# leaxer-ai/leaxer-qwen3-tts

Measured on AMD Instinct MI355X. Metric: real-time factor (24 kHz audio sec / wall sec), Qwen3-TTS-0.6B, higher is better.
Workload: dtype bf16 weights, fp32 activations/accumulate (codec decoder: fp16 hi/lo split operands, fp32 accumulate)

## Files before the change

### leaxer-qwen3-tts_amd/csrc/q3_common.h

```cpp
#pragma once
#include <hip/hip_runtime.h>
#include <stdint.h>
#include <string>

#include "../../include/q3tts.h"

typedef uint16_t bf16_t;

#define Q3_HIP_CHECK(expr)                                                                         \
    do {                                                                                           \
        hipError_t _e = (expr);                                                                    \
        if (_e != hipSuccess) throw q3::Error(std::string(#expr) + ": " + hipGetErrorString(_e));  \
    } while (0)

namespace q3 {

struct Error {
    std::string msg;
    explicit Error(std::string m) : msg(std::move(m)) {}
};

const char* knob(const char* name);
struct KnobScope {
    bool on = false;
// ... 28 lines not shown
    int ld_xn = 0;
    const float* bias = nullptr;
    const float* res = nullptr;
    int ldres = 0;
    float* out = nullptr;
    int ldo = 0;
    int M = 0, N = 0, K = 0;
    int epi = EPI_STORE;
    bool nt = false;
    const float* po = nullptr;
    const float* pm = nullptr;
    const float* pl = nullptr;
    int pS = 0, pchunk = 0, pn_new = 1, pslot_offset = 0, pheads = 0, pd = 0;
    const int* ppos_dev = nullptr;
    int ppos_scalar = 0;
};
void launch_gemv(const GemvArgs& a, hipStream_t s);
bool gemv_fast_path(const GemvArgs& a);
bool gemv16_ok(const GemvArgs& a);
void launch_gemv16(const GemvArgs& a, hipStream_t s);
void launch_pack_mfma_b(const bf16_t* W, bf16_t* P, int N, int K, hipStream_t s);
size_t packed_mfma_b_elems(int N, int K);
void register_packed_weight(const bf16_t* W, const bf16_t* P);
void unregister_packed_weight(const bf16_t* W);
const bf16_t* find_packed_weight(const bf16_t* W);

struct AttnArgs {
    const float* qkv = nullptr;
    int ld_qkv = 0;
    const float* ssq_in = nullptr; int ssq_nt = 0, ssq_K = 0; float ssq_eps = 0.f;
// ... 29 lines not shown
void launch_attn(const AttnArgs& a, hipStream_t s);
struct CpAttnOprojArgs {
    const float* qkv = nullptr; int ld_qkv = 0;
    float* kc = nullptr; float* vc = nullptr;
    int page_tokens = 0;
    int base = 0;
    const float* q_norm = nullptr; const float* k_norm = nullptr; float eps = 0.f;
    const float* rope_cos = nullptr; const float* rope_sin = nullptr;
    float scale = 0.f;
    int nq = 0, nkv = 0, d = 0;
    const bf16_t* W = nullptr; int K = 0, N = 0;
    float* x = nullptr; int ldx = 0;
};
bool cp_attn_oproj_ok(const CpAttnOprojArgs& a, int n_new);
void launch_cp_attn_oproj(const CpAttnOprojArgs& a, int n_new, hipStream_t s);
void launch_attn_combine(const AttnArgs& a, hipStream_t s);

struct GemmArgs {
    const bf16_t* W = nullptr;
    const bf16_t* W2 = nullptr;
    const bf16_t* xh = nullptr;
    const bf16_t* xl = nullptr;
    int ldx = 0;
    const float* res = nullptr; int ldres = 0;
    const float* bias = nullptr;
    float* out = nullptr; int ldo = 0;
    float* out2 = nullptr;
    bf16_t* oh = nullptr; bf16_t* ol = nullptr; int ldp = 0;
    int M = 0, N = 0, K = 0, epi = EPI_STORE;
    int slab_rows = 0;
// ... 141 lines not shown
```

### leaxer-qwen3-tts_amd/csrc/q3_decode_kernels.hip

```cpp
#include "q3_common.h"
#include "q3_wave_sort.h"
#include <algorithm>

namespace q3 {

#ifdef Q3_SAMPLE_PROF
__device__ long long g_kernel_prof[32];
void sample_prof_read(long long* out) { (void)hipMemcpyFromSymbol(out, HIP_SYMBOL(g_kernel_prof), sizeof(long long) * 32); }
#define KP_MARK(k) do { if (blockIdx.x == 0 && blockIdx.y == 0 && blockIdx.z == 0 && threadIdx.x == 0) g_kernel_prof[k] = wall_clock64(); } while (0)
#else
#define KP_MARK(k) do { } while (0)
#endif

#define Q3_DPP_XOR1 0xB1
#define Q3_DPP_XOR2 0x4E
#define Q3_DPP_ROR4 0x124
#define Q3_DPP_ROR8 0x128
#define Q3_DPP_BCAST15 0x142
#define Q3_DPP_BCAST31 0x143
template <int CTRL, int ROW_MASK>
static __device__ __forceinline__ float dpp_f(float oldv, float v) {
    return __builtin_bit_cast(float, __builtin_amdgcn_update_dpp(__builtin_bit_cast(int, oldv), __builtin_bit_cast(int, v), CTRL, ROW_MASK, 0xF, false));
}
template <int CTRL, int ROW_MASK>
// ... 183 lines not shown
    const int R = (a.N >= 4096 && a.epi != EPI_SWIGLU) ? 2 : 1;
    int grid = (a.N + 4 * R - 1) / (4 * R);
    if (grid > 2048) grid = 2048;
    if (grid < 1) grid = 1;
    if (R == 2) gemv_epi<MT, 2>(a, grid, s); else gemv_epi<MT, 1>(a, grid, s);
}


static __device__ __forceinline__ uint4 ldw_rt(const bf16_t* p, bool nt) {
    u32x4 v;
    if (nt) v = __builtin_nontemporal_load(reinterpret_cast<const u32x4*>(p));
    else v = *reinterpret_cast<const u32x4*>(p);
    return make_uint4(v.x, v.y, v.z, v.w);
}

template <int MT, int NCH, int RW, int EPI, bool NORM, bool COMB>
__global__ __launch_bounds__(256) void k_gemv1(const bf16_t* pW, const bf16_t* pW2, const float* px, const float* pgamma, const float* pepi,
                                                int pN, int pM, int pldx, int pldepi, int pnt, GemvArgs a) {
    constexpr int K = NCH * 512;
    const int lane = threadIdx.x & 63;
    const int wave = __builtin_amdgcn_readfirstlane(threadIdx.x >> 6);
    const int n0 = (blockIdx.x * 4 + wave) * RW;
    const int N = pN, M = pM;
    __shared__ float xs[COMB ? MT * K : 1];

    KP_MARK(30); KP_MARK(31);
    KP_MARK(8);
    uint4 w[RW][NCH], w2[RW][NCH];
#pragma unroll
    for (int r = 0; r < RW; ++r) {
        const int n = n0 + r < N ? n0 + r : N - 1;
#pragma unroll
        for (int c = 0; c < NCH; ++c) {
            w[r][c] = ldw_rt(pW + (size_t)n * K + c * 512 + lane * 8, pnt != 0);
            if (EPI == EPI_SWIGLU) w2[r][c] = ldw_rt(pW2 + (size_t)n * K + c * 512 + lane * 8, pnt != 0);
        }
    }
    __builtin_amdgcn_sched_barrier(0);
    float epi_in = 0.f;
    if (EPI == EPI_RESIDUAL || EPI == EPI_BIAS || EPI == EPI_BIAS_SILU) {
        if (lane < MT * RW) {
            const int m = lane / RW, n = n0 + lane % RW;
            if (m < M && n < N) epi_in = EPI == EPI_RESIDUAL ? pepi[(size_t)m * pldepi + n] : pepi[n];
        }
    }
    float xv[MT][NCH][8];
    if (COMB) {
        for (int k8 = threadIdx.x * 8; k8 < K; k8 += 2048) {
            const int head = k8 / a.pd, e0 = k8 % a.pd;
#pragma unroll
            for (int m = 0; m < MT; ++m) {
                if (m < M) {
                    const int bi = m / a.pn_new, inew = m % a.pn_new;
                    const int pos = (a.ppos_dev ? a.ppos_dev[a.pslot_offset + bi] : a.ppos_scalar) + inew;
                    int nact = pos / a.pchunk + 1;
                    if (nact > a.pS) nact = a.pS;
                    const size_t idx = ((size_t)m * a.pheads + head) * a.pS;
                    constexpr int CQ = 12;
                    float mx = -INFINITY, L = 0.f, O[8] = {0.f, 0.f, 0.f, 0.f, 0.f, 0.f, 0.f, 0.f};
                    for (int sp0 = 0; sp0 < nact; sp0 += CQ) {
                        float pmv[CQ], plv[CQ];
                        float4 o0[CQ], o1[CQ];
// ... 36 lines not shown
                xv[m][c][0] = x0.x; xv[m][c][1] = x0.y; xv[m][c][2] = x0.z; xv[m][c][3] = x0.w;
                xv[m][c][4] = x1.x; xv[m][c][5] = x1.y; xv[m][c][6] = x1.z; xv[m][c][7] = x1.w;
            }
    } else {
#pragma unroll
        for (int m = 0; m < MT; ++m)
#pragma unroll
            for (int c = 0; c < NCH; ++c) {
                const float* xr = px + (size_t)(m < M ? m : 0) * pldx + c * 512 + lane * 8;
                const float4 x0 = *reinterpret_cast<const float4*>(xr);
                const float4 x1 = *reinterpret_cast<const float4*>(xr + 4);
                xv[m][c][0] = x0.x; xv[m][c][1] = x0.y; xv[m][c][2] = x0.z; xv[m][c][3] = x0.w;
                xv[m][c][4] = x1.x; xv[m][c][5] = x1.y; xv[m][c][6] = x1.z; xv[m][c][7] = x1.w;
            }
    }
    float g[NORM ? NCH : 1][8];
    if (NORM) {
#pragma unroll
        for (int c = 0; c < NCH; ++c) {
            const float4 g0 = *reinterpret_cast<const float4*>(pgamma + c * 512 + lane * 8);
            const float4 g1 = *reinterpret_cast<const float4*>(pgamma + c * 512 + lane * 8 + 4);
            g[c][0] = g0.x; g[c][1] = g0.y; g[c][2] = g0.z; g[c][3] = g0.w; g[c][4] = g1.x; g[c][5] = g1.y; g[c][6] = g1.z; g[c][7] = g1.w;
        }
    }
    KP_MARK(9);
    __builtin_amdgcn_sched_barrier(0);
    if (NORM) {
#pragma unroll
        for (int m = 0; m < MT; ++m) {
            float ss = 0.f;
#pragma unroll
            for (int c = 0; c < NCH; ++c)
#pragma unroll
                for (int j = 0; j < 8; ++j) ss = fmaf(xv[m][c][j], xv[m][c][j], ss);
            ss = wave_sum(ss);
            const float inv = 1.0f / sqrtf(ss / (float)K + a.eps);
#pragma unroll
            for (int c = 0; c < NCH; ++c)
#pragma unroll
// ... 48 lines not shown
static int gemv1_rw(const GemvArgs& a) {
    int rw = a.N / 1024;
    if (rw < 1) rw = 1;
    if (rw > 4) rw = 4;
    if (a.epi == EPI_SWIGLU && rw > 3) rw = 3;
    if (a.K > 3072 && rw > 2) rw = 2;
    return rw;
}
bool gemv_fast_path(const GemvArgs& a) {
    if (a.M < 1 || a.M > 2) return false;
    if (a.K != 1024 && a.K != 2048 && a.K != 3072 && !(a.K == 6144 && a.M == 1)) return false;
    if (a.ldx % 4 != 0 && !a.po) return false;
    const bool norm = a.gamma != nullptr, comb = a.po != nullptr;
    if (comb && (norm || a.epi != EPI_RESIDUAL || a.pd % 8 != 0 || a.pheads * a.pd != a.K)) return false;
    if (norm && a.epi != EPI_STORE && a.epi != EPI_SWIGLU) return false;
    return true;
}

template <int MT, int NCH, int RW>
static void gemv1_launch(const GemvArgs& a, int grid, hipStream_t s) {
    const bool norm = a.gamma != nullptr, comb = a.po != nullptr;
#define Q3_G1(EPI, NORM, COMB) hipLaunchKernelGGL((k_gemv1<MT, NCH, RW, EPI, NORM, COMB>), dim3(grid), dim3(256), 0, s, a.W, a.W2, a.x, a.gamma, \
        (a.epi == EPI_RESIDUAL ? a.res : a.bias), a.N, a.M, a.ldx, a.ldres, (int)a.nt, a)
    if (comb) { Q3_G1(EPI_RESIDUAL, false, true); return; }
    switch (a.epi) {
    case EPI_STORE: if (norm) Q3_G1(EPI_STORE, true, false); else Q3_G1(EPI_STORE, false, false); break;
    case EPI_SWIGLU:
        if constexpr (RW <= 3) { if (norm) Q3_G1(EPI_SWIGLU, true, false); else Q3_G1(EPI_SWIGLU, false, false); }
        else throw Error("gemv: SwiGLU fast path takes at most 3 rows per wave");
        break;
    case EPI_RESIDUAL: Q3_G1(EPI_RESIDUAL, false, false); break;
    case EPI_BIAS: Q3_G1(EPI_BIAS, false, false); break;
    default: Q3_G1(EPI_BIAS_SILU, false, false); break;
    }
#undef Q3_G1
}
template <int MT, int NCH>
static void gemv1_rwsel(const GemvArgs& a, hipStream_t s) {
    const int rw = gemv1_rw(a);
    const int grid = (a.N + 4 * rw - 1) / (4 * rw);
    if (rw == 1) gemv1_launch<MT, NCH, 1>(a, grid, s);
    else if (rw == 2) gemv1_launch<MT, NCH, 2>(a, grid, s);
    else if constexpr (NCH <= 6) {
        if (rw == 3) gemv1_launch<MT, NCH, 3>(a, grid, s);
        else gemv1_launch<MT, NCH, 4>(a, grid, s);
    } else throw Error("gemv: K = 6144 fast path takes at most 2 rows per wave");
}
template <int MT>
static void gemv1_nch(const GemvArgs& a, hipStream_t s) {
    if (a.K == 1024) gemv1_rwsel<MT, 2>(a, s);
// ... 1366 lines not shown

void launch_cp_attn_oproj(const CpAttnOprojArgs& a, int n_new, hipStream_t s) {
    if (!cp_attn_oproj_ok(a, n_new)) throw Error("cp_attn_oproj: unsupported shape");
    const int U = a.base <= 4 ? 1 : (a.base <= 8 ? 2 : (a.base <= 12 ? 3 : 4));
    const dim3 grid((a.N + 3) / 4), block(1024);
#define Q3_CAO(NEW, UU) hipLaunchKernelGGL((k_cp_attn_oproj<NEW, UU>), grid, block, 0, s, a.W, a.qkv, (const float*)a.kc, (const float*)a.vc, (const float*)a.x, \
        a.rope_cos, a.rope_sin, (uint32_t)a.base | (uint32_t)a.page_tokens << 16, (uint32_t)a.N | (uint32_t)a.ldx << 16, a)
    if (n_new == 1) { if (U == 1) Q3_CAO(1, 1); else if (U == 2) Q3_CAO(1, 2); else if (U == 3) Q3_CAO(1, 3); else Q3_CAO(1, 4); }
    else { if (U == 1) Q3_CAO(2, 1); else if (U == 2) Q3_CAO(2, 2); else Q3_CAO(2, 3); }
#undef Q3_CAO
    Q3_HIP_CHECK(hipGetLastError());
}
bool cp_attn_oproj_ok(const CpAttnOprojArgs& a, int n_new) {
    return (n_new == 1 || (n_new == 2 && a.base <= 12)) && a.nq == 16 && a.nkv == 8 && a.d == 128 && a.K == 2048 && a.base >= 0 && a.base <= 16 &&
           a.base + n_new <= a.page_tokens && a.q_norm && a.k_norm && a.ld_qkv == 4096 && a.N >= 1 && a.N < 65536 && a.ldx < 65536 && a.page_tokens < 65536;
}

#define SAMP_MAXV 4096

static __device__ __forceinline__ uint64_t mix64(uint64_t z) {
    z += 0x9E3779B97F4A7C15ull;
    z = (z ^ (z >> 30)) * 0xBF58476D1CE4E5B9ull;
    z = (z ^ (z >> 27)) * 0x94D049BB133111EBull;
    return z ^ (z >> 31);
}
static __device__ __forceinline__ float rng_uniform_dev(uint64_t seed, uint32_t stream, uint32_t frame, uint32_t group) {
    uint64_t k = mix64(seed ^ mix64(((uint64_t)stream << 32) | frame));
    k = mix64(k + group);
    return (float)(k >> 40) * (1.0f / 16777216.0f);
}
// ... 635 lines not shown
```

### leaxer-qwen3-tts_amd/csrc/q3_engine.cpp

```cpp
#include "q3_engine.h"

#include <algorithm>
#include <atomic>
#include <cmath>
#include <cstdio>
#include <cstdlib>
#include <cstring>

namespace q3 {

static const int64_t TTS_BOS = 151672, TTS_EOS = 151673, TTS_PAD = 151671;
static const int64_t CODEC_BOS = 2149, CODEC_PAD = 2148, CODEC_THINK = 2154, CODEC_NOTHINK = 2155;
static const int64_t CODEC_THINK_BOS = 2156, CODEC_THINK_EOS = 2157, LANG_ENGLISH = 2050;

static uint64_t mix64(uint64_t z) {
    z += 0x9E3779B97F4A7C15ull;
    z = (z ^ (z >> 30)) * 0xBF58476D1CE4E5B9ull;
    z = (z ^ (z >> 27)) * 0x94D049BB133111EBull;
    return z ^ (z >> 31);
}
static uint64_t fnv1a(const std::string& s) {
    uint64_t h = 1469598103934665603ull;
    for (unsigned char ch : s) { h ^= ch; h *= 1099511628211ull; }
    return h;
// ... 136 lines not shown
    if (flags & Q3TTS_FLAG_TEST_HOOKS) knob_scope.enable();
    if (B < 1 || B > 1024) throw Error("max_batch out of range");
    if (kv_pool_tokens < 0) throw Error("kv_pool_tokens must be >= 0");
    if (c.cp_hidden < 0) throw Error("cp_hidden must be >= 0");
    if (c.cp_hidden == c.hidden) c.cp_hidden = 0;
    if (c.hidden % 8 || c.ffn % 8 || c.text_hidden % 8 || c.cp_ffn % 8 || cp_width() % 8) throw Error("hidden/ffn sizes must be multiples of 8");
    if (c.vocab > 4096 || c.sub_vocab > 4096) throw Error("codec vocabularies larger than 4096 are not supported");
    if (c.n_groups < 2 || c.n_groups > 32) throw Error("n_groups out of range");
    Q3_HIP_CHECK(hipSetDevice(device));
    if (const char* mr = knob("Q3TTS_MFMA_MIN_ROWS")) mfma_min_rows = std::max(3, atoi(mr));
    if (const char* sv = knob("Q3TTS_SEAM")) seam_on = atoi(sv) != 0;
    if (const char* sv = knob("Q3TTS_SEAM_SPIN")) seam_spin = std::max(1, atoi(sv));
    attn_keep_splits = knob("Q3TTS_ATTN_KEEP_SPLITS") != nullptr;
    if (const char* sv = knob("Q3TTS_ATTN_STREAM")) attn_stream = atoi(sv) != 0;
    if (const char* sv = knob("Q3TTS_ATTN_STREAM_ONE")) attn_stream_one = atoi(sv) != 0;
    null_stream = getenv("Q3TTS_NULL_STREAM") && getenv("Q3TTS_NULL_STREAM")[0] == '1';
    if (null_stream) { stream = nullptr; flags |= Q3TTS_FLAG_NO_GRAPH; }
    else if (const char* cm = knob("Q3TTS_STREAM_CU_MASK")) {
        const uint32_t pat = (uint32_t)strtoul(cm, nullptr, 16);
        if (pat == 0) throw Error("Q3TTS_STREAM_CU_MASK must be a non-zero hexadecimal CU pattern (a stream with no CU never runs)");
        uint32_t mask[8];
        for (int i = 0; i < 8; ++i) mask[i] = pat;
        Q3_HIP_CHECK(hipExtStreamCreateWithCUMask(&stream, 8, mask));
    }
    else {
        int lo = 0, hi = 0;
        Q3_HIP_CHECK(hipDeviceGetStreamPriorityRange(&lo, &hi));
        Q3_HIP_CHECK(hipStreamCreateWithPriority(&stream, hipStreamNonBlocking, hi));
    }
    Q3_HIP_CHECK(hipEventCreate(&ev0));
// ... 46 lines not shown
    x_cp1 = fm((size_t)B * H);
    if (cp_projected()) x_cpp = fm((size_t)std::max(rows_max, 16) * Hc);
    sum = fm((size_t)B * H);
    xp = fm((size_t)std::max(16, rows_max) * H);
    hn = fm((size_t)std::max(16, rows_max) * H);
    logits_p = fm((size_t)16 * std::max(c.vocab, c.sub_vocab));
    trailing_d = fm((size_t)B * max_trailing * H);
    tts_pad_d = fm(H);
    text_tmp = fm((size_t)16 * c.text_hidden);
    text_tmp2 = fm((size_t)16 * c.text_hidden);
    ldp = (std::max(std::max(H, AO), std::max(c.ffn, c.cp_ffn)) + 7) / 8 * 8;
    pl0h = (bf16_t*)dmalloc((size_t)rows_max * ldp * 2); pl0l = (bf16_t*)dmalloc((size_t)rows_max * ldp * 2);
    pl1h = (bf16_t*)dmalloc((size_t)rows_max * ldp * 2); pl1l = (bf16_t*)dmalloc((size_t)rows_max * ldp * 2);
    slab_d = fm((size_t)16 * rows_max * H);
    qkv_slab_d = fm((size_t)4 * rows_max * std::max(QKV, QKVp));
    {
        const size_t per_launch = (size_t)(std::max(std::max(c.ffn, c.cp_ffn), H) / 64 + 1) * 2 * 16;
        const size_t launches = (size_t)3 * ((size_t)c.n_layers + (size_t)(c.n_groups - 1) * c.cp_layers) + 8;
        seam_cnt_words = per_launch * launches;
        seam_cnt_d = (unsigned*)dmalloc(seam_cnt_words * sizeof(unsigned));
        Q3_HIP_CHECK(hipMemsetAsync(seam_cnt_d, 0, seam_cnt_words * sizeof(unsigned), stream));
        seam_gen_d = (unsigned*)dmalloc(64);
        Q3_HIP_CHECK(hipMemsetAsync(seam_gen_d, 0, 64, stream));
        ssq_a_d = fm((size_t)rows_max * 64);
        ssq_b_d = fm((size_t)rows_max * 64);
    }
    gu_slab_d = fm((size_t)2 * 8 * rows_max * std::max(c.ffn, c.cp_ffn));
    ids_d = (int64_t*)dmalloc(64 * sizeof(int64_t));
    tok_d = (int64_t*)dmalloc(sizeof(int64_t));
    codes_d = (int32_t*)dmalloc((size_t)B * max_frames_cap * c.n_groups * sizeof(int32_t));
// ... 249 lines not shown
        } else {
            GemvArgs g;
            g.W = w.qkv; g.x = x; g.ldx = ldx; g.gamma = w.in_norm; g.eps = W.eps; g.out = qkv; g.ldo = QKV;
            g.M = M; g.N = QKV; g.K = W.H; g.epi = EPI_STORE; g.nt = W.nt;
            launch_gemv(g, stream);
        }
        if (!mfma && nb == 1 && pos_dev == nullptr && slot_map == nullptr && W.n_splits == 1 && W.pages_per_slot == 1 && !W.kv_bf16 && !W.kv_round &&
            !(flags & Q3TTS_FLAG_NO_FUSED_CP)) {
            CpAttnOprojArgs f;
            const int ptok = 1 << W.page_shift;
            const size_t coff = (((size_t)slot_offset * W.L + l) * W.nkv) * ptok * W.d;
            f.qkv = qkv; f.ld_qkv = QKV; f.kc = W.kc + coff; f.vc = W.vc + coff; f.page_tokens = ptok; f.base = pos_scalar;
            f.q_norm = w.q_norm; f.k_norm = w.k_norm; f.eps = W.eps; f.rope_cos = W.rope_cos; f.rope_sin = W.rope_sin;
            f.scale = 1.0f / sqrtf((float)W.d); f.nq = W.nq; f.nkv = W.nkv; f.d = W.d; f.W = w.o; f.K = AO; f.N = W.H; f.x = x; f.ldx = ldx;
            if (cp_attn_oproj_ok(f, n_new)) {
                launch_cp_attn_oproj(f, n_new, stream);
                GemvArgs fg;
                fg.W = w.gate; fg.W2 = w.up; fg.x = x; fg.ldx = ldx; fg.gamma = w.post_norm; fg.eps = W.eps; fg.out = act; fg.ldo = W.ffn;
                fg.M = M; fg.N = W.ffn; fg.K = W.H; fg.epi = EPI_SWIGLU; fg.nt = W.nt;
                launch_gemv(fg, stream);
                GemvArgs dg;
                dg.W = w.down; dg.x = act; dg.ldx = W.ffn; dg.res = x; dg.ldres = ldx; dg.out = x; dg.ldo = ldx;
                dg.M = M; dg.N = W.H; dg.K = W.ffn; dg.epi = EPI_RESIDUAL; dg.nt = W.nt;
                launch_gemv(dg, stream);
                continue;
            }
        }
        AttnArgs a;
        a.qkv = qkv; a.ld_qkv = QKV; a.out = attn; a.ld_out = AO; a.kcache = W.kc; a.vcache = W.vc; a.kv_bf16 = W.kv_bf16; a.kv_round = W.kv_round;
        if (mfma) { a.qkv = qkv_slab_d; a.qkv_nslab = ks_q; a.qkv_slab_stride = (size_t)M * QKV; }
        if (seam && (l > 0 || planes_in)) { a.ssq_in = ssq_b_d; a.ssq_nt = NTH; a.ssq_K = W.H; a.ssq_eps = W.eps; }
        a.page_table = W.page_table; a.pages_per_slot = W.pages_per_slot; a.page_shift = W.page_shift; a.identity_pages = W.identity_pages;
        a.layer = l; a.n_layers = W.L; a.q_norm = w.q_norm; a.k_norm = w.k_norm; a.eps = W.eps;
        a.rope_cos = W.rope_cos; a.rope_sin = W.rope_sin; a.pos_dev = pos_dev; a.pos_scalar = pos_scalar;
        a.slot_offset = slot_offset; a.slot_map = slot_map; a.nb = nb; a.n_new = n_new; a.nq = W.nq; a.nkv = W.nkv; a.d = W.d;
        a.scale = 1.0f / sqrtf((float)W.d); a.window = 0; a.new_from_raw = 1;
        a.n_splits = W.n_splits; a.chunk = W.chunk; a.po = W.po; a.pm = W.pm; a.pl = W.pl;
        if (mfma && W.n_splits > 1 && W.identity_pages && !attn_keep_splits && (size_t)nb * W.nkv >= 256 && (W.pages_per_slot << W.page_shift) <= 512) {
// ... 42 lines not shown
                launch_gemm2(d, ks_d, 4, stream);
                continue;
            }
            launch_gemm2(d, ks_d, 4, stream);
            const bool last = l + 1 == W.L;
            const float* ng = last ? final_gamma : W.layers[l + 1].in_norm;
            launch_finish(x, ldx, slab_d, ks_d, (size_t)M * W.H, W.H, ng, last ? final_eps : W.eps, M, W.H, pl0h, pl0l, ldp,
                          last ? final_xn : nullptr, last ? final_ld_xn : 0, stream);
            continue;
        }
        GemvArgs o;
        o.W = w.o; o.x = attn; o.ldx = AO; o.res = x; o.ldres = ldx; o.out = x; o.ldo = ldx;
        o.M = M; o.N = W.H; o.K = AO; o.epi = EPI_RESIDUAL; o.nt = W.nt;
        o.po = W.po; o.pm = W.pm; o.pl = W.pl; o.pS = W.n_splits; o.pchunk = W.chunk; o.pn_new = n_new; o.pslot_offset = slot_offset;
        o.pheads = W.nq; o.pd = W.d; o.ppos_dev = pos_dev; o.ppos_scalar = pos_scalar;
        if (direct_rows) { o.po = nullptr; o.pm = nullptr; o.pl = nullptr; }
        else if (!gemv_fast_path(o)) {
            launch_attn_combine(a, stream);
            o.po = nullptr; o.pm = nullptr; o.pl = nullptr;
        }
        launch_gemv(o, stream);
        GemvArgs f;
        f.W = w.gate; f.W2 = w.up; f.x = x; f.ldx = ldx; f.gamma = w.post_norm; f.eps = W.eps; f.out = act; f.ldo = W.ffn;
        f.M = M; f.N = W.ffn; f.K = W.H; f.epi = EPI_SWIGLU; f.nt = W.nt;
        launch_gemv(f, stream);
        GemvArgs d;
        d.W = w.down; d.x = act; d.ldx = W.ffn; d.res = x; d.ldres = ldx; d.out = x; d.ldo = ldx;
        d.M = M; d.N = W.H; d.K = W.ffn; d.epi = EPI_RESIDUAL; d.nt = W.nt;
        launch_gemv(d, stream);
    }
    return mfma && final_gamma != nullptr;
}

int Engine::head_proj(const bf16_t* Wm, const float* x, int ldx, const float* gamma, float eps, float* xn_out, int ld_xn,
                      float* out, int ldo, int M, int N, int K, bool nt, bool planes_ready, int plane_row0, int plane_row_stride, float* slab_out) {
    if (planes_ready || (M >= mfma_min_rows && K % 128 == 0 && K <= 4096)) {
        if (!planes_ready) {
            launch_finish(const_cast<float*>(x), ldx, nullptr, 0, 0, 0, gamma, eps, M, K, pl0h, pl0l, ldp, xn_out, ld_xn, stream);
            plane_row0 = 0; plane_row_stride = 1;
        }
        GemmArgs g;
        g.W = Wm; g.xh = pl0h + (size_t)plane_row0 * ldp; g.xl = pl0l + (size_t)plane_row0 * ldp; g.ldx = ldp * plane_row_stride;
        g.out = out; g.ldo = ldo; g.M = M; g.N = N; g.K = K; g.epi = EPI_STORE; g.nt = nt;
// ... 824 lines not shown
```

### leaxer-qwen3-tts_amd/csrc/q3_engine.h

```cpp
#pragma once
#include <functional>
#include <memory>
#include <string>
#include <unordered_map>
#include <vector>

#include "q3_common.h"
#include "q3_kvpool.h"

namespace q3 {

enum TensorKind { TK_W = 0, TK_NORM = 1, TK_BIAS = 2, TK_SCALE = 3, TK_SNAKE = 4 };

struct Tensor {
    std::string name;
    int64_t shape[4] = {0, 0, 0, 0};
    int ndim = 0;
    int kind = TK_W;
    bool bf16 = false;
    void* dev = nullptr;
    int64_t numel = 0;
    float synth_std = 0.02f;
};

// ... 174 lines not shown
    float* cp_project(float* rows, int ld, int M);
    std::vector<const bf16_t*> cp_head, cp_embed_w;

    int rows_max = 0, max_trailing = 0, max_frames_cap = 0;
    int mfma_min_rows = 12;
    float *x_talk = nullptr, *qkv = nullptr, *attn = nullptr, *act = nullptr, *logits_t = nullptr, *logits_cp = nullptr;
    float *x_cp = nullptr, *x_cp1 = nullptr, *sum = nullptr, *xp = nullptr, *hn = nullptr, *logits_p = nullptr;
    float *trailing_d = nullptr, *tts_pad_d = nullptr, *text_tmp = nullptr, *text_tmp2 = nullptr;
    int64_t* ids_d = nullptr;
    bf16_t *pl0h = nullptr, *pl0l = nullptr, *pl1h = nullptr, *pl1l = nullptr;
    int ldp = 0;
    float* slab_d = nullptr;
    float* gu_slab_d = nullptr;
    float* cp_logit_slab_d = nullptr;
    float* qkv_slab_d = nullptr;
    unsigned* seam_cnt_d = nullptr; size_t seam_cnt_words = 0, seam_cnt_used = 0;
    unsigned* seam_gen_d = nullptr;
    float *ssq_a_d = nullptr, *ssq_b_d = nullptr;
    bool seam_step = false;
    bool seam_on = true;
    bool attn_stream = true;
    bool attn_stream_one = true;
    bool attn_keep_splits = false;
    int seam_spin = 512;
    int32_t* codes_d = nullptr;
    int32_t* codes_scratch_d = nullptr;
    int32_t* talker_pos_d = nullptr;
    int* slot_map_d = nullptr;
    float* logits_g = nullptr;
    SlotState* st_d = nullptr;
// ... 23 lines not shown
```

Before: 35.90.

## Split o-proj by KV head into partial sums folded into gate/up GEMV prologue

Attention plus o-projection (both the code-predictor fused path and the talker split-combine path) now run with one block per KV-head slice of K and a column chunk. Each writes a per-head partial output vector instead of doing the full K reduction per column inside one block. The following SwiGLU gate/up GEMV gains a prologue that sums the 8 partials with the residual, writes the mid residual for the down projection, and applies RMSNorm. This aims to raise parallelism in the M=1 decode o-proj and remove its serial full-K reduction. The cost is extra partial-buffer traffic and every gate/up block redundantly re-reading the partials.

```diff
diff --git a/leaxer-qwen3-tts_amd/csrc/q3_common.h b/leaxer-qwen3-tts_amd/csrc/q3_common.h
--- a/leaxer-qwen3-tts_amd/csrc/q3_common.h
+++ b/leaxer-qwen3-tts_amd/csrc/q3_common.h
@@ -66,6 +66,8 @@
     int pS = 0, pchunk = 0, pn_new = 1, pslot_offset = 0, pheads = 0, pd = 0;
     const int* ppos_dev = nullptr;
     int ppos_scalar = 0;
+    const float* psum = nullptr;
+    float* xmid = nullptr;
 };
 void launch_gemv(const GemvArgs& a, hipStream_t s);
 bool gemv_fast_path(const GemvArgs& a);
@@ -125,6 +127,9 @@
 };
 bool cp_attn_oproj_ok(const CpAttnOprojArgs& a, int n_new);
 void launch_cp_attn_oproj(const CpAttnOprojArgs& a, int n_new, hipStream_t s);
+void launch_cp_attn_kvh(const CpAttnOprojArgs& a, int n_new, float* part, hipStream_t s);
+bool oproj_kvh_ok(const GemvArgs& a);
+void launch_oproj_kvh(const GemvArgs& a, float* part, hipStream_t s);
 void launch_attn_combine(const AttnArgs& a, hipStream_t s);
 
 struct GemmArgs {
diff --git a/leaxer-qwen3-tts_amd/csrc/q3_decode_kernels.hip b/leaxer-qwen3-tts_amd/csrc/q3_decode_kernels.hip
--- a/leaxer-qwen3-tts_amd/csrc/q3_decode_kernels.hip
+++ b/leaxer-qwen3-tts_amd/csrc/q3_decode_kernels.hip
@@ -221,7 +221,7 @@
     return make_uint4(v.x, v.y, v.z, v.w);
 }
 
-template <int MT, int NCH, int RW, int EPI, bool NORM, bool COMB>
+template <int MT, int NCH, int RW, int EPI, bool NORM, bool COMB, bool PSUM = false>
 __global__ __launch_bounds__(256) void k_gemv1(const bf16_t* pW, const bf16_t* pW2, const float* px, const float* pgamma, const float* pepi,
                                                 int pN, int pM, int pldx, int pldepi, int pnt, GemvArgs a) {
     constexpr int K = NCH * 512;
@@ -229,7 +229,7 @@
     const int wave = __builtin_amdgcn_readfirstlane(threadIdx.x >> 6);
     const int n0 = (blockIdx.x * 4 + wave) * RW;
     const int N = pN, M = pM;
-    __shared__ float xs[COMB ? MT * K : 1];
+    __shared__ float xs[(COMB || PSUM) ? MT * K : 1];
 
     KP_MARK(30); KP_MARK(31);
     KP_MARK(8);
@@ -251,8 +251,56 @@
             if (m < M && n < N) epi_in = EPI == EPI_RESIDUAL ? pepi[(size_t)m * pldepi + n] : pepi[n];
         }
     }
+    float g[NORM ? NCH : 1][8];
+    auto load_gamma = [&]() {
+#pragma unroll
+        for (int c = 0; c < NCH; ++c) {
+            const float4 g0 = *reinterpret_cast<const float4*>(pgamma + c * 512 + lane * 8);
+            const float4 g1 = *reinterpret_cast<const float4*>(pgamma + c * 512 + lane * 8 + 4);
+            g[c][0] = g0.x; g[c][1] = g0.y; g[c][2] = g0.z; g[c][3] = g0.w; g[c][4] = g1.x; g[c][5] = g1.y; g[c][6] = g1.z; g[c][7] = g1.w;
+        }
+    };
     float xv[MT][NCH][8];
-    if (COMB) {
+    if (PSUM) {
+        constexpr int NI = K / 1024, NP = 8;
+        static_assert(K % 1024 == 0, "PSUM: K must be a multiple of 1024");
+        float4 xin[MT][NI], pin[MT][NI][NP];
+#pragma unroll
+        for (int m = 0; m < MT; ++m) {
+            const int mr = m < M ? m : 0;
+#pragma unroll
+            for (int i = 0; i < NI; ++i) {
+                const int k4 = i * 1024 + threadIdx.x * 4;
+                xin[m][i] = *reinterpret_cast<const float4*>(px + (size_t)mr * pldx + k4);
+#pragma unroll
+                for (int h = 0; h < NP; ++h) pin[m][i][h] = *reinterpret_cast<const float4*>(a.psum + ((size_t)h * M + mr) * K + k4);
+            }
+        }
+        if (NORM) load_gamma();
+        __builtin_amdgcn_sched_barrier(0);
+#pragma unroll
+        for (int m = 0; m < MT; ++m)
+#pragma unroll
+            for (int i = 0; i < NI; ++i) {
+                const int k4 = i * 1024 + threadIdx.x * 4;
+                float4 ps = pin[m][i][0];
+#pragma unroll
+                for (int h = 1; h < NP; ++h) { ps.x += pin[m][i][h].x; ps.y += pin[m][i][h].y; ps.z += pin[m][i][h].z; ps.w += pin[m][i][h].w; }
+                const float4 v = make_float4(xin[m][i].x + ps.x, xin[m][i].y + ps.y, xin[m][i].z + ps.z, xin[m][i].w + ps.w);
+                *reinterpret_cast<float4*>(&xs[m * K + k4]) = v;
+                if (m < M && (k4 / 4) % gridDim.x == blockIdx.x) *reinterpret_cast<float4*>(a.xmid + (size_t)m * K + k4) = v;
+            }
+        __syncthreads();
+#pragma unroll
+        for (int m = 0; m < MT; ++m)
+#pragma unroll
+            for (int c = 0; c < NCH; ++c) {
+                const float4 x0 = *reinterpret_cast<const float4*>(&xs[m * K + c * 512 + lane * 8]);
+                const float4 x1 = *reinterpret_cast<const float4*>(&xs[m * K + c * 512 + lane * 8 + 4]);
+                xv[m][c][0] = x0.x; xv[m][c][1] = x0.y; xv[m][c][2] = x0.z; xv[m][c][3] = x0.w;
+                xv[m][c][4] = x1.x; xv[m][c][5] = x1.y; xv[m][c][6] = x1.z; xv[m][c][7] = x1.w;
+            }
+    } else if (COMB) {
         for (int k8 = threadIdx.x * 8; k8 < K; k8 += 2048) {
             const int head = k8 / a.pd, e0 = k8 % a.pd;
 #pragma unroll
@@ -319,15 +367,7 @@
                 xv[m][c][4] = x1.x; xv[m][c][5] = x1.y; xv[m][c][6] = x1.z; xv[m][c][7] = x1.w;
             }
     }
-    float g[NORM ? NCH : 1][8];
-    if (NORM) {
-#pragma unroll
-        for (int c = 0; c < NCH; ++c) {
-            const float4 g0 = *reinterpret_cast<const float4*>(pgamma + c * 512 + lane * 8);
-            const float4 g1 = *reinterpret_cast<const float4*>(pgamma + c * 512 + lane * 8 + 4);
-            g[c][0] = g0.x; g[c][1] = g0.y; g[c][2] = g0.z; g[c][3] = g0.w; g[c][4] = g1.x; g[c][5] = g1.y; g[c][6] = g1.z; g[c][7] = g1.w;
-        }
-    }
+    if (NORM && !PSUM) load_gamma();
     KP_MARK(9);
     __builtin_amdgcn_sched_barrier(0);
     if (NORM) {
@@ -406,15 +446,22 @@
     const bool norm = a.gamma != nullptr, comb = a.po != nullptr;
     if (comb && (norm || a.epi != EPI_RESIDUAL || a.pd % 8 != 0 || a.pheads * a.pd != a.K)) return false;
     if (norm && a.epi != EPI_STORE && a.epi != EPI_SWIGLU) return false;
+    if (a.psum && (!norm || a.epi != EPI_SWIGLU || a.K % 1024 != 0 || a.K > 2048 || a.xmid == nullptr || a.xn_out || gemv1_rw(a) > 3)) return false;
     return true;
 }
 
 template <int MT, int NCH, int RW>
 static void gemv1_launch(const GemvArgs& a, int grid, hipStream_t s) {
     const bool norm = a.gamma != nullptr, comb = a.po != nullptr;
-#define Q3_G1(EPI, NORM, COMB) hipLaunchKernelGGL((k_gemv1<MT, NCH, RW, EPI, NORM, COMB>), dim3(grid), dim3(256), 0, s, a.W, a.W2, a.x, a.gamma, \
+#define Q3_G1(EPI, NORM, COMB) Q3_G1P(EPI, NORM, COMB, false)
+#define Q3_G1P(EPI, NORM, COMB, PSUM) hipLaunchKernelGGL((k_gemv1<MT, NCH, RW, EPI, NORM, COMB, PSUM>), dim3(grid), dim3(256), 0, s, a.W, a.W2, a.x, a.gamma, \
         (a.epi == EPI_RESIDUAL ? a.res : a.bias), a.N, a.M, a.ldx, a.ldres, (int)a.nt, a)
     if (comb) { Q3_G1(EPI_RESIDUAL, false, true); return; }
+    if (a.psum) {
+        if constexpr (RW <= 3 && NCH % 2 == 0 && NCH <= 4) Q3_G1P(EPI_SWIGLU, true, false, true);
+        else throw Error("gemv: partial-sum prologue not built for this shape");
+        return;
+    }
     switch (a.epi) {
     case EPI_STORE: if (norm) Q3_G1(EPI_STORE, true, false); else Q3_G1(EPI_STORE, false, false); break;
     case EPI_SWIGLU:
@@ -426,6 +473,7 @@
     default: Q3_G1(EPI_BIAS_SILU, false, false); break;
     }
 #undef Q3_G1
+#undef Q3_G1P
 }
 template <int MT, int NCH>
 static void gemv1_rwsel(const GemvArgs& a, hipStream_t s) {
@@ -1822,6 +1870,270 @@
 bool cp_attn_oproj_ok(const CpAttnOprojArgs& a, int n_new) {
     return (n_new == 1 || (n_new == 2 && a.base <= 12)) && a.nq == 16 && a.nkv == 8 && a.d == 128 && a.K == 2048 && a.base >= 0 && a.base <= 16 &&
            a.base + n_new <= a.page_tokens && a.q_norm && a.k_norm && a.ld_qkv == 4096 && a.N >= 1 && a.N < 65536 && a.ldx < 65536 && a.page_tokens < 65536;
+}
+
+#define KVH_COLS 32
+static __device__ __forceinline__ void kvh_load_w(uint4 (&w)[4], const bf16_t* pW, int N, int K, int n0, int k0, int lane) {
+#pragma unroll
+    for (int i = 0; i < 4; ++i) {
+        int n = n0 + 2 * i + (lane >> 5);
+        n = n < N ? n : N - 1;
+        w[i] = ldw_rt(pW + (size_t)n * K + k0 + (lane & 31) * 8, false);
+    }
+}
+static __device__ __forceinline__ void kvh_gemv_store(const uint4 (&w)[4], const float* xs, float* out, int N, int n0, int lane) {
+    const float* xr = xs + (lane & 31) * 8;
+    const float4 x0 = *reinterpret_cast<const float4*>(xr), x1 = *reinterpret_cast<const float4*>(xr + 4);
+    const float xv[8] = { x0.x, x0.y, x0.z, x0.w, x1.x, x1.y, x1.z, x1.w };
+#pragma unroll
+    for (int i = 0; i < 4; ++i) {
+        const uint32_t wu[4] = { w[i].x, w[i].y, w[i].z, w[i].w };
+        float s = 0.f;
+#pragma unroll
+        for (int j = 0; j < 4; ++j) { s = fmaf(xv[2 * j], bf_lo(wu[j]), s); s = fmaf(xv[2 * j + 1], bf_hi(wu[j]), s); }
+        s = row_sum16(s);
+        s += wave_xor_lane_f<16>(s, lane);
+        const int n = n0 + 2 * i + (lane >> 5);
+        if ((lane & 31) == 0 && n < N) out[n] = s;
+    }
+}
+
+template <int NEW, int U>
+__global__ __launch_bounds__(256) void k_cp_attn_kvh(const bf16_t* pW, const float* pqkv, const float* pkc, const float* pvc, float* ppart,
+                                                     const float* pcos, const float* psin, uint32_t pk0, uint32_t pk1, CpAttnOprojArgs a) {
+    const int pbase = (int)(pk0 & 0xFFFFu), ppage_tokens = (int)(pk0 >> 16), pN = (int)pk1;
+    constexpr int LDQ = 4096;
+    constexpr int D = 128, HALF = 64, EPL = 8, G = 2, NKV = 8, NQ = 16, K = 2048, KS = G * D;
+    const int tid = threadIdx.x, lane = tid & 63;
+    const int wave = __builtin_amdgcn_readfirstlane(tid >> 6);
+    const int kvh = blockIdx.x % NKV, chunk = blockIdx.x / NKV;
+    const int head = kvh * G + (wave & 1);
+    const int base = pbase;
+    const int n0 = chunk * KVH_COLS + wave * 8;
+
+    __shared__ float q_s[G][NEW][D];
+    __shared__ float knew[G][NEW][D];
+    __shared__ float vnew[G][NEW][D];
+    __shared__ float attn_s[NEW][KS];
+
+    uint4 w[4];
+    kvh_load_w(w, pW, pN, K, n0, kvh * KS, lane);
+    __builtin_amdgcn_sched_barrier(0);
+
+    if (wave < G) {
+        struct VecOps { float x0, x1, v0, v1, n0, n1, cs, sn; };
+        constexpr int NVEC = 2 * NEW;
+        VecOps vec[NVEC];
+#pragma unroll
+        for (int v = 0; v < NVEC; ++v) {
+            const bool is_q = v < NEW;
+            const int j = is_q ? v : v - NEW;
+            const float* rowp = pqkv + (size_t)j * LDQ;
+            const float* src = rowp + (is_q ? head * D : (NQ + kvh) * D);
+            const float* vs = rowp + (NQ + NKV + kvh) * D;
+            const float* nw = is_q ? a.q_norm : a.k_norm;
+            vec[v].x0 = src[lane]; vec[v].x1 = src[lane + HALF];
+            vec[v].v0 = vs[lane]; vec[v].v1 = vs[lane + HALF];
+            vec[v].n0 = nw[lane]; vec[v].n1 = nw[lane + HALF];
+            vec[v].cs = pcos[(size_t)(base + j) * HALF + lane]; vec[v].sn = psin[(size_t)(base + j) * HALF + lane];
+        }
+        const int tg = lane >> 4, sub = lane & 15;
+        float kr[U][EPL], vr[U][EPL];
+#pragma unroll
+        for (int u = 0; u < U; ++u) {
+            int t = tg + 4 * u;
+            t = t < base ? t : base - 1;
+            t = t > 0 ? t : 0;
+            const size_t off = ((size_t)kvh * ppage_tokens + t) * D + sub * EPL;
+            const float4 k0 = *reinterpret_cast<const float4*>(pkc + off), k1 = *reinterpret_cast<const float4*>(pkc + off + 4);
+            const float4 v0 = *reinterpret_cast<const float4*>(pvc + off), v1 = *reinterpret_cast<const float4*>(pvc + off + 4);
+            kr[u][0] = k0.x; kr[u][1] = k0.y; kr[u][2] = k0.z; kr[u][3] = k0.w; kr[u][4] = k1.x; kr[u][5] = k1.y; kr[u][6] = k1.z; kr[u][7] = k1.w;
+            vr[u][0] = v0.x; vr[u][1] = v0.y; vr[u][2] = v0.z; vr[u][3] = v0.w; vr[u][4] = v1.x; vr[u][5] = v1.y; vr[u][6] = v1.z; vr[u][7] = v1.w;
+        }
+        __builtin_amdgcn_sched_barrier(0);
+
+#pragma unroll
+        for (int v = 0; v < NVEC; ++v) {
+            const bool is_q = v < NEW;
+            const int j = is_q ? v : v - NEW;
+            const float ss = wave_sum(vec[v].x0 * vec[v].x0 + vec[v].x1 * vec[v].x1);
+            const float rr = 1.0f / sqrtf(ss / (float)D + a.eps);
+            const float x0 = vec[v].n0 * (vec[v].x0 * rr), x1 = vec[v].n1 * (vec[v].x1 * rr);
+            const float y0 = x0 * vec[v].cs + (-x1) * vec[v].sn;
+            const float y1 = x1 * vec[v].cs + x0 * vec[v].sn;
+            if (is_q) { q_s[wave][j][lane] = y0; q_s[wave][j][lane + HALF] = y1; }
+            else {
+                knew[wave][j][lane] = y0; knew[wave][j][lane + HALF] = y1;
+                vnew[wave][j][lane] = vec[v].v0; vnew[wave][j][lane + HALF] = vec[v].v1;
+                if (chunk == 0 && wave == 0) {
+                    const size_t off = ((size_t)kvh * a.page_tokens + base + j) * D;
+                    a.kc[off + lane] = y0; a.kc[off + lane + HALF] = y1;
+                    a.vc[off + lane] = vec[v].v0; a.vc[off + lane + HALF] = vec[v].v1;
+                }
+            }
+        }
+        __builtin_amdgcn_fence(__ATOMIC_RELEASE, "wavefront");
+        __builtin_amdgcn_wave_barrier();
+        __builtin_amdgcn_fence(__ATOMIC_ACQUIRE, "wavefront");
+
+        float kn[NEW][EPL], vn[NEW][EPL];
+#pragma unroll
+        for (int j = 0; j < NEW; ++j)
+#pragma unroll
+            for (int e = 0; e < EPL; ++e) { kn[j][e] = knew[wave][j][sub * EPL + e]; vn[j][e] = vnew[wave][j][sub * EPL + e]; }
+#pragma unroll
+        for (int inew = 0; inew < NEW; ++inew) {
+            float qr[EPL];
+#pragma unroll
+            for (int e = 0; e < EPL; ++e) qr[e] = q_s[wave][inew][sub * EPL + e];
+            float sc[U + NEW];
+#pragma unroll
+            for (int u = 0; u < U; ++u) {
+                float sdot = 0.f;
+#pragma unroll
+                for (int e = 0; e < EPL; ++e) sdot = fmaf(qr[e], kr[u][e], sdot);
+                sdot = row_sum16(sdot) * a.scale;
+                sc[u] = tg + 4 * u < base ? sdot : -INFINITY;
+            }
+#pragma unroll
+            for (int j = 0; j < NEW; ++j) {
+                float sdot = 0.f;
+#pragma unroll
+                for (int e = 0; e < EPL; ++e) sdot = fmaf(qr[e], kn[j][e], sdot);
+                sdot = row_sum16(sdot) * a.scale;
+                sc[U + j] = (j <= inew && (j & 3) == tg) ? sdot : -INFINITY;
+            }
+            float mx = -INFINITY;
+#pragma unroll
+            for (int i = 0; i < U + NEW; ++i) mx = fmaxf(mx, sc[i]);
+            float l = 0.f, o[EPL];
+#pragma unroll
+            for (int e = 0; e < EPL; ++e) o[e] = 0.f;
+#pragma unroll
+            for (int u = 0; u < U; ++u) {
+                const float pw = mx == -INFINITY ? 0.f : __expf(sc[u] - mx);
+                l += pw;
+#pragma unroll
+                for (int e = 0; e < EPL; ++e) o[e] = fmaf(pw, tg + 4 * u < base ? vr[u][e] : 0.f, o[e]);
+            }
+#pragma unroll
+            for (int j = 0; j < NEW; ++j) {
+                const float pw = mx == -INFINITY ? 0.f : __expf(sc[U + j] - mx);
+                l += pw;
+#pragma unroll
+                for (int e = 0; e < EPL; ++e) o[e] = fmaf(pw, vn[j][e], o[e]);
+            }
+            const float mall = wave_max(mx);
+            const float wgt = mx == -INFINITY ? 0.f : __expf(mx - mall);
+            l *= wgt;
+#pragma unroll
+            for (int e = 0; e < EPL; ++e) o[e] *= wgt;
+            l += wave_xor_lane_f<16>(l, lane);
+            l += wave_xor_lane_f<32>(l, lane);
+#pragma unroll
+            for (int e = 0; e < EPL; ++e) { o[e] += wave_xor_lane_f<16>(o[e], lane); o[e] += wave_xor_lane_f<32>(o[e], lane); }
+            if (tg == 0) {
+                const float il = 1.0f / l;
+                float* dst = &attn_s[inew][wave * D + sub * EPL];
+                *reinterpret_cast<float4*>(dst) = make_float4(o[0] * il, o[1] * il, o[2] * il, o[3] * il);
+                *reinterpret_cast<float4*>(dst + 4) = make_float4(o[4] * il, o[5] * il, o[6] * il, o[7] * il);
+            }
+        }
+    }
+    __syncthreads();
+#pragma unroll
+    for (int m = 0; m < NEW; ++m) kvh_gemv_store(w, attn_s[m], ppart + ((size_t)kvh * NEW + m) * pN, pN, n0, lane);
+}
+
+void launch_cp_attn_kvh(const CpAttnOprojArgs& a, int n_new, float* part, hipStream_t s) {
+    if (!cp_attn_oproj_ok(a, n_new) || part == nullptr) throw Error("cp_attn_kvh: unsupported shape");
+    const int U = a.base <= 4 ? 1 : (a.base <= 8 ? 2 : (a.base <= 12 ? 3 : 4));
+    const dim3 grid(((a.N + KVH_COLS - 1) / KVH_COLS) * 8), block(256);
+#define Q3_CAK(NEW, UU) hipLaunchKernelGGL((k_cp_attn_kvh<NEW, UU>), grid, block, 0, s, a.W, a.qkv, (const float*)a.kc, (const float*)a.vc, part, \
+        a.rope_cos, a.rope_sin, (uint32_t)a.base | (uint32_t)a.page_tokens << 16, (uint32_t)a.N, a)
+    if (n_new == 1) { if (U == 1) Q3_CAK(1, 1); else if (U == 2) Q3_CAK(1, 2); else if (U == 3) Q3_CAK(1, 3); else Q3_CAK(1, 4); }
+    else { if (U == 1) Q3_CAK(2, 1); else if (U == 2) Q3_CAK(2, 2); else Q3_CAK(2, 3); }
+#undef Q3_CAK
+    Q3_HIP_CHECK(hipGetLastError());
+}
+
+__global__ __launch_bounds__(256) void k_oproj_kvh(const bf16_t* pW, const float* ppo, const float* ppm, const float* ppl, float* ppart,
+                                                   const int* ppos_dev, int ppos, int pS, int pchunk, int pN, int pK, int pd) {
+    constexpr int NKV = 8, G = 2, KS = 256, SG = 8, CQ = 8;
+    const int tid = threadIdx.x, lane = tid & 63;
+    const int wave = __builtin_amdgcn_readfirstlane(tid >> 6);
+    const int kvh = blockIdx.x % NKV, chunk = blockIdx.x / NKV;
+    const int n0 = chunk * KVH_COLS + wave * 8;
+    __shared__ float sm[SG][32], sl[SG][32];
+    __shared__ float so[SG][32][8];
+    __shared__ float xs[KS];
+
+    const int pos = ppos_dev ? ppos_dev[0] : ppos;
+    uint4 w[4];
+    kvh_load_w(w, pW, pN, pK, n0, kvh * KS, lane);
+    __builtin_amdgcn_sched_barrier(0);
+    int nact = pos / pchunk + 1;
+    nact = nact < pS ? nact : pS;
+    const int eg = tid & 31, sg = tid >> 5;
+    const int head = kvh * G + (eg >> 4), e0 = (eg & 15) * 8;
+    const size_t idx = (size_t)head * pS;
+    float pmv[CQ], plv[CQ];
+    float4 o0[CQ], o1[CQ];
+#pragma unroll
+    for (int q = 0; q < CQ; ++q) {
+        int sp = sg + SG * q;
+        sp = sp < nact ? sp : nact - 1;
+        pmv[q] = ppm[idx + sp]; plv[q] = ppl[idx + sp];
+        o0[q] = *reinterpret_cast<const float4*>(ppo + (idx + sp) * pd + e0);
+        o1[q] = *reinterpret_cast<const float4*>(ppo + (idx + sp) * pd + e0 + 4);
+    }
+    __builtin_amdgcn_sched_barrier(0);
+    float mx = -INFINITY;
+#pragma unroll
+    for (int q = 0; q < CQ; ++q) if (sg + SG * q < nact) mx = fmaxf(mx, pmv[q]);
+    float L = 0.f, O[8] = {0.f, 0.f, 0.f, 0.f, 0.f, 0.f, 0.f, 0.f};
+#pragma unroll
+    for (int q = 0; q < CQ; ++q) {
+        const float wgt = sg + SG * q < nact ? __expf(pmv[q] - mx) : 0.f;
+        L += wgt * plv[q];
+        O[0] += wgt * o0[q].x; O[1] += wgt * o0[q].y; O[2] += wgt * o0[q].z; O[3] += wgt * o0[q].w;
+        O[4] += wgt * o1[q].x; O[5] += wgt * o1[q].y; O[6] += wgt * o1[q].z; O[7] += wgt * o1[q].w;
+    }
+    sm[sg][eg] = mx; sl[sg][eg] = L;
+    *reinterpret_cast<float4*>(&so[sg][eg][0]) = make_float4(O[0], O[1], O[2], O[3]);
+    *reinterpret_cast<float4*>(&so[sg][eg][4]) = make_float4(O[4], O[5], O[6], O[7]);
+    __syncthreads();
+    if (tid < 32) {
+        float m = sm[0][eg];
+#pragma unroll
+        for (int g = 1; g < SG; ++g) m = fmaxf(m, sm[g][eg]);
+        float l = 0.f, o[8] = {0.f, 0.f, 0.f, 0.f, 0.f, 0.f, 0.f, 0.f};
+#pragma unroll
+        for (int g = 0; g < SG; ++g) {
+            const float wgt = sm[g][eg] == -INFINITY ? 0.f : __expf(sm[g][eg] - m);
+            l += wgt * sl[g][eg];
+#pragma unroll
+            for (int j = 0; j < 8; ++j) o[j] += wgt * so[g][eg][j];
+        }
+        const float il = 1.0f / l;
+        float* dst = &xs[eg * 8];
+        *reinterpret_cast<float4*>(dst) = make_float4(o[0] * il, o[1] * il, o[2] * il, o[3] * il);
+        *reinterpret_cast<float4*>(dst + 4) = make_float4(o[4] * il, o[5] * il, o[6] * il, o[7] * il);
+    }
+    __syncthreads();
+    kvh_gemv_store(w, xs, ppart + (size_t)kvh * pN, pN, n0, lane);
+}
+
+bool oproj_kvh_ok(const GemvArgs& a) {
+    return a.M == 1 && a.po && a.pm && a.pl && a.pheads == 16 && a.pd == 128 && a.K == 2048 && a.pS >= 1 && a.pS <= 64 && a.pchunk >= 1 &&
+           a.pn_new == 1 && a.N >= 1 && a.epi == EPI_RESIDUAL && a.gamma == nullptr;
+}
+void launch_oproj_kvh(const GemvArgs& a, float* part, hipStream_t s) {
+    if (!oproj_kvh_ok(a) || part == nullptr) throw Error("oproj_kvh: unsupported shape");
+    const dim3 grid(((a.N + KVH_COLS - 1) / KVH_COLS) * 8), block(256);
+    hipLaunchKernelGGL(k_oproj_kvh, grid, block, 0, s, a.W, a.po, a.pm, a.pl, part, a.ppos_dev ? a.ppos_dev + a.pslot_offset : nullptr, a.ppos_scalar,
+                       a.pS, a.pchunk, a.N, a.K, a.pd);
+    Q3_HIP_CHECK(hipGetLastError());
 }
 
 #define SAMP_MAXV 4096
diff --git a/leaxer-qwen3-tts_amd/csrc/q3_engine.cpp b/leaxer-qwen3-tts_amd/csrc/q3_engine.cpp
--- a/leaxer-qwen3-tts_amd/csrc/q3_engine.cpp
+++ b/leaxer-qwen3-tts_amd/csrc/q3_engine.cpp
@@ -174,6 +174,7 @@
     attn_keep_splits = knob("Q3TTS_ATTN_KEEP_SPLITS") != nullptr;
     if (const char* sv = knob("Q3TTS_ATTN_STREAM")) attn_stream = atoi(sv) != 0;
     if (const char* sv = knob("Q3TTS_ATTN_STREAM_ONE")) attn_stream_one = atoi(sv) != 0;
+    if (const char* sv = knob("Q3TTS_KVH_OPROJ")) kvh_oproj = atoi(sv) != 0;
     null_stream = getenv("Q3TTS_NULL_STREAM") && getenv("Q3TTS_NULL_STREAM")[0] == '1';
     if (null_stream) { stream = nullptr; flags |= Q3TTS_FLAG_NO_GRAPH; }
     else if (const char* cm = knob("Q3TTS_STREAM_CU_MASK")) {
@@ -250,6 +251,8 @@
     pl1h = (bf16_t*)dmalloc((size_t)rows_max * ldp * 2); pl1l = (bf16_t*)dmalloc((size_t)rows_max * ldp * 2);
     slab_d = fm((size_t)16 * rows_max * H);
     qkv_slab_d = fm((size_t)4 * rows_max * std::max(QKV, QKVp));
+    oproj_part_d = fm((size_t)8 * 2 * std::max(H, Hc));
+    xmid_d = fm((size_t)2 * std::max(H, Hc));
     {
         const size_t per_launch = (size_t)(std::max(std::max(c.ffn, c.cp_ffn), H) / 64 + 1) * 2 * 16;
         const size_t launches = (size_t)3 * ((size_t)c.n_layers + (size_t)(c.n_groups - 1) * c.cp_layers) + 8;
@@ -529,14 +532,21 @@
             f.q_norm = w.q_norm; f.k_norm = w.k_norm; f.eps = W.eps; f.rope_cos = W.rope_cos; f.rope_sin = W.rope_sin;
             f.scale = 1.0f / sqrtf((float)W.d); f.nq = W.nq; f.nkv = W.nkv; f.d = W.d; f.W = w.o; f.K = AO; f.N = W.H; f.x = x; f.ldx = ldx;
             if (cp_attn_oproj_ok(f, n_new)) {
-                launch_cp_attn_oproj(f, n_new, stream);
                 GemvArgs fg;
                 fg.W = w.gate; fg.W2 = w.up; fg.x = x; fg.ldx = ldx; fg.gamma = w.post_norm; fg.eps = W.eps; fg.out = act; fg.ldo = W.ffn;
                 fg.M = M; fg.N = W.ffn; fg.K = W.H; fg.epi = EPI_SWIGLU; fg.nt = W.nt;
-                launch_gemv(fg, stream);
                 GemvArgs dg;
                 dg.W = w.down; dg.x = act; dg.ldx = W.ffn; dg.res = x; dg.ldres = ldx; dg.out = x; dg.ldo = ldx;
                 dg.M = M; dg.N = W.H; dg.K = W.ffn; dg.epi = EPI_RESIDUAL; dg.nt = W.nt;
+                fg.psum = oproj_part_d; fg.xmid = xmid_d;
+                if (kvh_oproj && gemv_fast_path(fg)) {
+                    launch_cp_attn_kvh(f, n_new, oproj_part_d, stream);
+                    dg.res = xmid_d; dg.ldres = W.H;
+                } else {
+                    fg.psum = nullptr; fg.xmid = nullptr;
+                    launch_cp_attn_oproj(f, n_new, stream);
+                }
+                launch_gemv(fg, stream);
                 launch_gemv(dg, stream);
                 continue;
             }
@@ -609,19 +619,30 @@
         o.M = M; o.N = W.H; o.K = AO; o.epi = EPI_RESIDUAL; o.nt = W.nt;
         o.po = W.po; o.pm = W.pm; o.pl = W.pl; o.pS = W.n_splits; o.pchunk = W.chunk; o.pn_new = n_new; o.pslot_offset = slot_offset;
         o.pheads = W.nq; o.pd = W.d; o.ppos_dev = pos_dev; o.ppos_scalar = pos_scalar;
-        if (direct_rows) { o.po = nullptr; o.pm = nullptr; o.pl = nullptr; }
-        else if (!gemv_fast_path(o)) {
-            launch_attn_combine(a, stream);
-            o.po = nullptr; o.pm = nullptr; o.pl = nullptr;
-        }
-        launch_gemv(o, stream);
         GemvArgs f;
         f.W = w.gate; f.W2 = w.up; f.x = x; f.ldx = ldx; f.gamma = w.post_norm; f.eps = W.eps; f.out = act; f.ldo = W.ffn;
         f.M = M; f.N = W.ffn; f.K = W.H; f.epi = EPI_SWIGLU; f.nt = W.nt;
-        launch_gemv(f, stream);
         GemvArgs d;
         d.W = w.down; d.x = act; d.ldx = W.ffn; d.res = x; d.ldres = ldx; d.out = x; d.ldo = ldx;
         d.M = M; d.N = W.H; d.K = W.ffn; d.epi = EPI_RESIDUAL; d.nt = W.nt;
+        bool kvh = false;
+        if (!direct_rows && kvh_oproj && W.nkv == 8 && W.nq == 16 && oproj_kvh_ok(o) && gemv_fast_path(o)) {
+            f.psum = oproj_part_d; f.xmid = xmid_d;
+            kvh = gemv_fast_path(f);
+            if (!kvh) { f.psum = nullptr; f.xmid = nullptr; }
+        }
+        if (kvh) {
+            launch_oproj_kvh(o, oproj_part_d, stream);
+            d.res = xmid_d; d.ldres = W.H;
+        } else {
+            if (direct_rows) { o.po = nullptr; o.pm = nullptr; o.pl = nullptr; }
+            else if (!gemv_fast_path(o)) {
+                launch_attn_combine(a, stream);
+                o.po = nullptr; o.pm = nullptr; o.pl = nullptr;
+            }
+            launch_gemv(o, stream);
+        }
+        launch_gemv(f, stream);
         launch_gemv(d, stream);
     }
     return mfma && final_gamma != nullptr;
diff --git a/leaxer-qwen3-tts_amd/csrc/q3_engine.h b/leaxer-qwen3-tts_amd/csrc/q3_engine.h
--- a/leaxer-qwen3-tts_amd/csrc/q3_engine.h
+++ b/leaxer-qwen3-tts_amd/csrc/q3_engine.h
@@ -212,6 +212,8 @@
     float* gu_slab_d = nullptr;
     float* cp_logit_slab_d = nullptr;
     float* qkv_slab_d = nullptr;
+    float *oproj_part_d = nullptr, *xmid_d = nullptr;
+    bool kvh_oproj = true;
     unsigned* seam_cnt_d = nullptr; size_t seam_cnt_words = 0, seam_cnt_used = 0;
     unsigned* seam_gen_d = nullptr;
     float *ssq_a_d = nullptr, *ssq_b_d = nullptr;
```

New measurement: 38.23, median of 6. 6.5% higher.
